# JNP-Solutions/Slacken

Hardware: AMD Instinct MI355X
Metric: classify_throughput_150bp_standard224scale (higher is better)
Workload: dtype u64

## Files before the change

### slacken_amd/csrc/lane.hip

```cpp
#include "engine.h"

#include <algorithm>
#include <cstddef>
#include <cstdio>
#include <cstdlib>

namespace slk {

#ifndef SLK_LANE_LW
#define SLK_LANE_LW 4
#endif
constexpr int LW = SLK_LANE_LW;
constexpr int QCAP = 128;
#ifndef SLK_SBLK
#define SLK_SBLK 5
#endif
constexpr int SBLK = SLK_SBLK;
#ifndef SLK_OMAP
#define SLK_OMAP 12
#endif
constexpr int OMAP = SLK_OMAP;
constexpr int OMAP_CNT_BITS = 10;
constexpr uint32_t OMAP_CNT_MASK = (1u << OMAP_CNT_BITS) - 1;

struct __attribute__((aligned(16))) LaneLds {
  uint64_t q_key[QCAP];
  uint32_t q_meta[QCAP];
  uint64_t stash[128];
  uint32_t found[64];
  uint4 sbuf[(SBLK - 1) * 64];
  uint32_t omap[OMAP * 64];
  uint32_t o_flags[64];
  uint64_t rb[64];
  uint16_t q_ord[QCAP];
};

#ifdef SLK_TUNING
#define SLK_TUNE(...) __VA_ARGS__
#define SLK_TUNE_ON(bit) ((dbg & (bit)) != 0)
#else
#define SLK_TUNE(...)
#define SLK_TUNE_ON(bit) false
#endif

#ifndef SLK_PROBE_NT
#define SLK_PROBE_NT 0
#endif
__device__ __forceinline__ ulonglong2 SLK_PROBE_LOAD(const ulonglong2 *p) {
#if SLK_PROBE_NT
  ulonglong2 v;
  v.x = __builtin_nontemporal_load(&p->x);
  v.y = __builtin_nontemporal_load(&p->y);
  return v;
#else
  return *p;
#endif
}

template <bool LONG>
__device__ __forceinline__ void fold_hit(LaneLds *L, uint32_t *ocnt, bool in, uint32_t meta, int32_t taxon) {
  if (in && taxon != 0) {
    const int owner = meta & 63;
    const int32_t kmers = (int32_t)((meta >> 7) & 0x1FFF);
    if (meta & 64) atomicAdd(&L->o_flags[owner], 1u);
    uint32_t slot = (uint32_t)(((uint64_t)((uint32_t)taxon * 0x9E3779B1u) * (uint32_t)OMAP) >> 32);
    int p = 0;
    if (LONG) {
      for (; p < OMAP; p++) {
        uint32_t old = atomicCAS(&L->omap[slot * 64 + owner], 0u, (uint32_t)taxon);
        if (old == 0u || old == (uint32_t)taxon) { atomicAdd(&ocnt[slot * 64 + owner], (uint32_t)kmers); break; }
        slot = (slot + 1 == (uint32_t)OMAP) ? 0u : slot + 1;
      }
    } else {
      const uint32_t fresh = ((uint32_t)taxon << OMAP_CNT_BITS) | (uint32_t)kmers;
      for (; p < OMAP; p++) {
        uint32_t old = atomicCAS(&L->omap[slot * 64 + owner], 0u, fresh);
        if (old == 0u) break;
        if ((old >> OMAP_CNT_BITS) == (uint32_t)taxon) { atomicAdd(&L->omap[slot * 64 + owner], (uint32_t)kmers); break; }
        slot = (slot + 1 == (uint32_t)OMAP) ? 0u : slot + 1;
      }
    }
    if (p == OMAP) atomicOr(&L->o_flags[owner], 0x80000000u);
  }
}

constexpr int PG = 64 / LPB;
template <bool HITS, bool LONG>
__device__ __forceinline__ int probe_batch(LaneLds *L, uint32_t *ocnt, const TableView &T, int qhead, int qn, int cnt, int lane, int dbg,
                                           int32_t *hit_meta, int32_t *hit_taxon) {
  const uint64_t NO_TAG = ~0ULL;
  const bool in = lane < cnt;
  const int qi = (qhead + lane) & (QCAP - 1);
  const uint64_t key = L->q_key[qi];
  const uint32_t meta = L->q_meta[qi];
  const uint32_t ord = HITS ? L->q_ord[qi] : 0u;
  const uint64_t h = fmix64(key);
  uint32_t home;
  uint64_t rem_hi;
  table_slot(T.g, h, home, rem_hi);
  uint4 st;
  const uint32_t disp = (meta >> 20) & 255;
  st.x = table_bucket(T.g, home, disp);
  st.y = 0;
  const uint64_t tag = in ? (rem_hi + disp) : NO_TAG;
  st.z = (uint32_t)tag; st.w = (uint32_t)(tag >> 32);
  ((uint4 *)L->stash)[lane] = st;
  L->found[lane] = 0;
  wave_sync();
  const int g = lane / LPB, c = lane % LPB;
  const uint64_t tmask = (1ULL << T.g.taxon_bits) - 1;
  const char *cellbase = (const char *)T.cells + c * 16;
  ulonglong2 cell[LPB];
#pragma unroll
  for (int s = 0; s < LPB; s++) {
    uint32_t bkt = ((const uint4 *)L->stash)[s * PG + g].x;
    SLK_TUNE(if (dbg & 4) bkt &= 1023u;)
    cell[s] = SLK_PROBE_LOAD((const ulonglong2 *)(cellbase + ((uint64_t)bkt << BUCKET_SHIFT)));
  }
  constexpr uint64_t GROUP_LSB = LPB == 4 ? 0x1111111111111111ULL : 0x0101010101010101ULL;
  int requeued = 0;
#pragma unroll
  for (int s = 0; s < LPB; s++) {
    const uint2 tg = *(const uint2 *)&((const uint4 *)L->stash)[s * PG + g].z;
    const uint64_t want = ((uint64_t)tg.y << 32) | tg.x;
    const bool act = want != NO_TAG;
    const bool e0 = cell[s].x == 0, e1 = cell[s].y == 0;
    const bool m0 = act && !e0 && cell_tag(T.g, cell[s].x) == want;
    const bool m1 = act && !e1 && cell_tag(T.g, cell[s].y) == want;
    if (m0 || m1) L->found[s * PG + g] = (uint32_t)((m0 ? cell[s].x : cell[s].y) & tmask);
    const bool closed = T.g.flag != 0 && c == 0 && (cell[s].x & T.g.flag) == 0;
    const uint64_t B = __ballot(m0 || m1 || e0 || e1 || !act || closed);
    uint64_t any = B;
#pragma unroll
    for (int i = 1; i < LPB; i <<= 1) any |= any >> i;
    if ((any & GROUP_LSB) != GROUP_LSB) {
      const int qj = (qhead + s * PG + g) & (QCAP - 1);
      const uint32_t m_old = L->q_meta[qj];
      const bool again = c == 0 && ((B >> (g * LPB)) & ((1u << LPB) - 1)) == 0 && (int)((m_old >> 20) & 255) < T.max_disp;
      const uint64_t k_old = L->q_key[qj];
      const uint16_t o_old = HITS ? L->q_ord[qj] : (uint16_t)0;
      const uint64_t R = __ballot(again);
      wave_sync();
      if (again) {
        const int slot = (qhead + qn + requeued + __builtin_amdgcn_mbcnt_hi((uint32_t)(R >> 32), __builtin_amdgcn_mbcnt_lo((uint32_t)R, 0))) & (QCAP - 1);
        L->q_key[slot] = k_old;
        L->q_meta[slot] = m_old + (1u << 20);
        if (HITS) L->q_ord[slot] = o_old;
      }
      requeued += __popcll(R);
    }
  }
  wave_sync();
  const int32_t taxon = (int32_t)L->found[lane];
  if (!SLK_TUNE_ON(2)) fold_hit<LONG>(L, ocnt, in, meta, taxon);
  if (HITS && in) {
    const uint64_t at = L->rb[meta & 63] + ord;
    hit_taxon[at] = ext_taxon(T, taxon);
    hit_meta[at] = pack_meta((int32_t)((meta >> 7) & 0x1FFF), 1, (meta >> 6) & 1);
  }
  wave_sync();
  return requeued;
}

#ifndef SLK_STREAM_NT
#define SLK_STREAM_NT 0
#endif
#ifndef SLK_APPLY_ROWS
#define SLK_APPLY_ROWS 4
#endif
template <class T> __device__ __forceinline__ T SLK_STREAM_LOAD(const T *p) {
#if SLK_STREAM_NT
  return __builtin_nontemporal_load(p);
#else
  return *p;
#endif
}
template <class T> __device__ __forceinline__ void SLK_STREAM_STORE(T *p, T v) {
#if SLK_STREAM_NT
  __builtin_nontemporal_store(v, p);
#else
  *p = v;
#endif
}

__device__ __forceinline__ uint32_t shard_owner(uint64_t key, uint32_t ns) {
  const uint64_t h = fmix64(key);
  return (ns & (ns - 1)) == 0 ? (uint32_t)(h & (ns - 1)) : (uint32_t)(h % ns);
}
__device__ __forceinline__ uint64_t side_load(const ShardIO &S, uint64_t batch, int lane) {
  const uint64_t i = batch * 64 + (uint64_t)lane;
  return i < S.side_n ? (uint64_t)SLK_STREAM_LOAD(&S.side_keys[i]) : 0;
}
__device__ __forceinline__ void side_probe(LaneLds *L, const TableView &T, const ShardIO &S, int lane, uint64_t batch, uint64_t key, int dbg) {
  const uint64_t base = batch * 64;
  if (base >= S.side_n) return;
  const uint64_t i = base + (uint64_t)lane;
  const bool in = i < S.side_n;
  const uint64_t h = fmix64(key);
  uint32_t home;
  uint64_t rem_hi;
  table_slot(T.g, h, home, rem_hi);
  const uint64_t tag = in ? rem_hi : ~0ULL;
  uint4 st;
  st.x = home; st.y = 0; st.z = (uint32_t)tag; st.w = (uint32_t)(tag >> 32);
  ((uint4 *)L->stash)[lane] = st;
  L->found[lane] = 0;
  wave_sync();
  const int g = lane / LPB, c = lane % LPB;
  const uint64_t tmask = (1ULL << T.g.taxon_bits) - 1;
  const char *cellbase = (const char *)T.cells + c * 16;
  ulonglong2 cell[LPB];
#pragma unroll
  for (int s = 0; s < LPB; s++) {
    uint32_t bkt = ((const uint4 *)L->stash)[s * PG + g].x;
    SLK_TUNE(if (dbg & 4) bkt &= 1023u;)
    cell[s] = SLK_PROBE_LOAD((const ulonglong2 *)(cellbase + ((uint64_t)bkt << BUCKET_SHIFT)));
  }
  uint32_t unresolved = 0;
#pragma unroll
  for (int s = 0; s < LPB; s++) {
    const uint2 tg = *(const uint2 *)&((const uint4 *)L->stash)[s * PG + g].z;
    const uint64_t want = ((uint64_t)tg.y << 32) | tg.x;
    const bool act = want != ~0ULL;
    const bool e0 = cell[s].x == 0, e1 = cell[s].y == 0;
    const bool m0 = act && !e0 && cell_tag(T.g, cell[s].x) == want;
    const bool m1 = act && !e1 && cell_tag(T.g, cell[s].y) == want;
    if (m0 || m1) L->found[s * PG + g] = (uint32_t)((m0 ? cell[s].x : cell[s].y) & tmask);
    const bool closed = T.g.flag != 0 && c == 0 && (cell[s].x & T.g.flag) == 0;
    const uint64_t B = __ballot(m0 || m1 || e0 || e1 || !act || closed);
    if (((B >> (g * LPB)) & ((1u << LPB) - 1)) == 0) unresolved |= 1u << s;
  }
  wave_sync();
  int32_t taxon = (int32_t)L->found[lane];
  const uint32_t ur = (uint32_t)__shfl((int)unresolved, (lane % PG) * LPB);
  if (in && ((ur >> (lane / PG)) & 1)) {
    for (int d = 1; d <= T.max_disp; d++) {
      const ulonglong2 *b = (const ulonglong2 *)(T.cells + ((uint64_t)table_bucket(T.g, home, (uint32_t)d) * CELLS));
      const uint64_t want = rem_hi | (uint64_t)d;
      bool has_empty = false, closed = false;
      int32_t hit = 0;
#pragma unroll
      for (int q = 0; q < LPB; q++) {
        const ulonglong2 v = b[q];
        has_empty |= (v.x == 0) | (v.y == 0);
        if (q == 0) closed = T.g.flag != 0 && (v.x & T.g.flag) == 0;
        if (v.x != 0 && cell_tag(T.g, v.x) == want) hit = (int32_t)(v.x & tmask);
        if (v.y != 0 && cell_tag(T.g, v.y) == want) hit = (int32_t)(v.y & tmask);
      }
      if (hit) { taxon = hit; break; }
      if (has_empty || closed) break;
    }
  }
  if (in && !SLK_TUNE_ON(128)) SLK_STREAM_STORE(&S.side_out[i], ext_taxon(T, taxon));
  wave_sync();
}

template <bool HITS>
__device__ __forceinline__ void apply_rows(LaneLds *L, const ApplyJob &J, int lane, uint64_t row0, uint32_t nrows) {
  const uint32_t ns = (uint32_t)J.n_shards;
  constexpr int U = SLK_APPLY_ROWS;
  for (uint32_t b = 0; b < nrows; b += U) {
    uint64_t at[U];
    bool in[U];
#pragma unroll
    for (int u = 0; u < U; u++) {
      in[u] = false;
      at[u] = 0;
      if (b + u < nrows) {
        uint32_t off = 0;
        for (uint32_t sh = 0; sh < ns; sh++) {
          const uint4 e = J.batch_log[(row0 + b + u) * ns + sh];
          const uint32_t cnt = e.z;
          if (cnt == 0) continue;
          if ((uint32_t)lane >= off && (uint32_t)lane < off + cnt) {
            in[u] = true;
            const uint32_t i = (uint32_t)lane - off;
            at[u] = (uint64_t)sh * J.cap + (i < e.w ? e.x + i : e.y + (i - e.w));
          }
          off += cnt;
        }
      }
    }
    uint32_t meta[U];
    int32_t taxon[U];
#pragma unroll
    for (int u = 0; u < U; u++) {
      meta[u] = in[u] ? SLK_STREAM_LOAD(&J.send_meta[at[u]]) : 0u;
      taxon[u] = in[u] ? SLK_STREAM_LOAD(&J.taxa[at[u]]) : 0;
    }
#pragma unroll
    for (int u = 0; u < U; u++) {
      if (b + u < nrows) {
        int32_t t = taxon[u];
        if (in[u]) {
          if (HITS) {
            const uint64_t hat = L->rb[meta[u] & 63] + (meta[u] >> 20);
            J.A.span_taxon[hat] = t;
            J.A.span_meta[hat] = pack_meta((int32_t)((meta[u] >> 7) & 0x1FFF), 1, (meta[u] >> 6) & 1);
          }
          if (J.to_dense != nullptr && t > 0) t = t < J.n_to_dense ? J.to_dense[t] : 0;
        }
        fold_hit<false>(L, nullptr, in[u], meta[u], t);
      }
    }
    wave_sync();
  }
}

template <bool HITS>
__device__ __forceinline__ void emit_batch(LaneLds *L, const FusedArgs &A, const ShardIO &S, const ApplyJob &J, int qhead, int cnt, int lane,
                                           uint64_t row, uint64_t tile, uint32_t &ch_pos, uint32_t &ch_end, uint32_t &side_j, uint64_t &side_key, int dbg) {
  SLK_TUNE(if (dbg & 256) return;)
  const bool in = lane < cnt;
  const int qi = (qhead + lane) & (QCAP - 1);
  const uint64_t key = L->q_key[qi];
  const uint32_t meta = L->q_meta[qi] | (HITS ? (uint32_t)L->q_ord[qi] << 20 : 0u);
  const uint32_t ns = (uint32_t)S.n_shards;
  const uint32_t g = ns == 1 ? 0u : shard_owner(key, ns);
  uint32_t mycount = 0, rank = 0;
  for (uint32_t sh = 0; sh < ns; sh++) {
    const uint64_t m = __ballot(in && g == sh);
    if ((uint32_t)lane == sh) mycount = (uint32_t)__popcll(m);
    if (g == sh) rank = __builtin_amdgcn_mbcnt_hi((uint32_t)(m >> 32), __builtin_amdgcn_mbcnt_lo((uint32_t)m, 0));
  }
  const uint32_t pos = ch_pos, room = ch_end - ch_pos;
  const bool need = (uint32_t)lane < ns && mycount > room;
  unsigned long long got = 0;
  if (need) got = atomicAdd(&S.cursors[lane], (unsigned long long)S.chunk);
  if (side_j < S.side_per_tile) {
    const uint64_t batch = tile * S.side_per_tile + side_j;
    const uint64_t k_now = side_key;
    side_j++;
    if (side_j < S.side_per_tile) side_key = side_load(S, batch + 1, lane);
    side_probe(L, A.T, S, lane, batch, k_now, dbg);
  }
  uint32_t fresh = 0xFFFFFFFFu;
  if (need) {
    if (got + S.chunk <= S.cap) fresh = (uint32_t)got;
    else atomicOr(A.status, 2);
  }
  if ((uint32_t)lane < ns) {
    S.batch_log[row * ns + (uint32_t)lane] = make_uint4(pos, fresh, mycount, room);
    if (need) { ch_pos = fresh == 0xFFFFFFFFu ? 0u : fresh + (mycount - room); ch_end = fresh == 0xFFFFFFFFu ? 0u : fresh + S.chunk; }
    else ch_pos = pos + mycount;
  }
  const uint32_t gpos = (uint32_t)__shfl((int)pos, (int)g), groom = (uint32_t)__shfl((int)room, (int)g), gfresh = (uint32_t)__shfl((int)fresh, (int)g);
  if (in) {
    const bool tail = rank >= groom;
    if ((!tail || gfresh != 0xFFFFFFFFu) && !SLK_TUNE_ON(32)) {
      const uint64_t at = (uint64_t)g * S.cap + (tail ? gfresh + (rank - groom) : gpos + rank);
      SLK_STREAM_STORE(&S.send_keys[at], (int64_t)key);
      SLK_STREAM_STORE(&S.send_meta[at], meta);
    }
  }
  wave_sync();
}

#ifndef SLK_PACKED_STREAM
#define SLK_PACKED_STREAM 1
#endif
#ifndef SLK_PACK_ROUNDS
#define SLK_PACK_ROUNDS 2
#endif
constexpr uint32_t PACK_MAX_SPAN = 10880;
constexpr uint32_t PACK_WORDS = PACK_MAX_SPAN / 16 + 1;
constexpr int PACK_LOADS = (PACK_MAX_SPAN + 1023) / 1024;
static_assert((size_t)PACK_WORDS * 6 <= (size_t)(SBLK - 1) * 64 * 16, "the packed tile lives in the lane-wise stream's LDS slots");
__device__ __forceinline__ void pack16(const uint4 v, uint32_t &codes, uint32_t &valid) {
  const uint32_t VM = (1u << 1) | (1u << 3) | (1u << 7) | (1u << 20) | (1u << 21);
  const uint32_t w[4] = {v.x, v.y, v.z, v.w};
  codes = 0; valid = 0;
#pragma unroll
  for (int d = 0; d < 4; d++) {
    uint32_t t = (w[d] >> 1) & 0x03030303u;
    t ^= (t >> 1) & 0x01010101u;
    t = (t | (t >> 6) | (t >> 12) | (t >> 18)) & 0xFFu;
    codes |= t << (8 * d);
#pragma unroll
    for (int b = 0; b < 4; b++) {
      const uint32_t c = (w[d] >> (8 * b)) & 0xFFu;
      const uint32_t ok = (((c & 0xC0u) == 0x40u) ? 1u : 0u) & (VM >> (c & 31u));
      valid |= (ok & 1u) << (4 * d + b);
    }
  }
}
__device__ __forceinline__ uint2 packed_take(const uint32_t *pcodes, const uint16_t *pvalid, uint32_t s) {
  const uint32_t wi = s >> 4, bo = s & 15u;
  const uint64_t c64 = (uint64_t)pcodes[wi] | ((uint64_t)pcodes[wi + 1] << 32);
  const uint32_t v32 = (uint32_t)pvalid[wi] | ((uint32_t)pvalid[wi + 1] << 16);
  return make_uint2((uint32_t)(c64 >> (2 * bo)), (v32 >> bo) & 0xFFFFu);
}

#ifndef SLK_LANE_WPS
#define SLK_LANE_WPS 0
#endif
#if SLK_LANE_WPS > 0
#define LANE_BOUNDS __launch_bounds__(LW * 64, SLK_LANE_WPS)
#else
#define LANE_BOUNDS __launch_bounds__(LW * 64) __attribute__((amdgpu_waves_per_eu(4)))
#endif

__device__ __forceinline__ int route_by_length(uint64_t len, uint32_t long_max, uint32_t b0, uint32_t b1, uint32_t b2, uint32_t seg_min_len,
                                               uint32_t wave_min, uint32_t wave_ratio_q10) {
  if (long_max != 0 && len <= long_max) return (len > b0) + (len > b1) + (len > b2);
  if (seg_min_len != 0 && len >= seg_min_len) return HandOn::SEG;
  int c = HandOn::WAVE_CLASSES - 1;
  for (uint64_t b = ((uint64_t)wave_min * wave_ratio_q10) >> 10; c > 0 && len >= b; b = (b * wave_ratio_q10) >> 10) c--;
  return HandOn::WAVE0 + c;
}
__device__ __attribute__((noinline)) void hand_on(unsigned long long *hdr, uint32_t *lists, uint64_t stride, uint64_t long_cap, uint32_t long_max,
                                                  uint32_t b0, uint32_t b1, uint32_t b2, uint32_t seg_min_len, uint32_t wave_min,
                                                  uint32_t wave_ratio_q10, const uint64_t *offsets, const uint64_t *mate_offsets, bool dfr,
                                                  bool too_long, uint64_t r, int lane, bool from_long) {
  const uint64_t DM = __ballot(dfr);
  int route = from_long ? HandOn::LATE : HandOn::REST;
  if (!from_long && dfr && too_long) {
    uint64_t len = offsets[r + 1] - offsets[r];
    if (mate_offsets) len += mate_offsets[r + 1] - mate_offsets[r];
    route = route_by_length(len, long_max, b0, b1, b2, seg_min_len, wave_min, wave_ratio_q10);
  }
  if (!from_long && lane == 0) atomicAdd(&hdr[HandOn::HANDED], (unsigned long long)__popcll(DM));
  for (int l = from_long ? HandOn::LATE : 0; l <= HandOn::LATE; l++) {
    const uint64_t M = __ballot(dfr && route == l);
    if (M == 0) continue;
    const int leader = __ffsll((long long)M) - 1;
    unsigned long long at = 0;
    if (lane == leader) at = atomicAdd(&hdr[HandOn::count_word(l)], (unsigned long long)__popcll(M));
    at = readlane64(at, leader);
    if (dfr && route == l)
      lists[HandOn::list_at(l, stride, long_cap) + at + __builtin_amdgcn_mbcnt_hi((uint32_t)(M >> 32), __builtin_amdgcn_mbcnt_lo((uint32_t)M, 0))] = (uint32_t)r;
  }
}

__global__ void __launch_bounds__(256) route_kernel(FusedArgs A) {
  constexpr int PER = 8, NL = HandOn::LISTS;
  __shared__ uint32_t cnt[NL];
  __shared__ unsigned long long base[NL];
  const uint64_t chunk = 256 * PER, chunks = (A.R + chunk - 1) / chunk;
  for (uint64_t c = blockIdx.x; c < chunks; c += gridDim.x) {
    if (threadIdx.x < NL) cnt[threadIdx.x] = 0;
    __syncthreads();
    int route[PER];
    uint32_t rank[PER];
#pragma unroll
    for (int j = 0; j < PER; j++) {
      const uint64_t r = c * chunk + (uint64_t)j * 256 + threadIdx.x;
      route[j] = -1;
      rank[j] = 0;
      if (r < A.R) {
        uint64_t len = A.offsets[r + 1] - A.offsets[r];
        if (A.mate_offsets) len += A.mate_offsets[r + 1] - A.mate_offsets[r];
        route[j] = len <= 1000 ? (int)HandOn::SHORT : route_by_length(len, A.long_max, A.long_bound[0], A.long_bound[1], A.long_bound[2],
                                                                      A.seg_min_len, A.wave_min, A.wave_ratio_q10);
        rank[j] = atomicAdd(&cnt[route[j]], 1u);
      }
    }
    __syncthreads();
    if (threadIdx.x < NL && cnt[threadIdx.x] != 0)
      base[threadIdx.x] = atomicAdd(&A.hand_hdr[HandOn::count_word((int)threadIdx.x)], (unsigned long long)cnt[threadIdx.x]);
    if (threadIdx.x == 0) {
      uint32_t handed = 0;
      for (int l = 0; l < NL; l++) if (l != HandOn::SHORT) handed += cnt[l];
      if (handed) atomicAdd(&A.hand_hdr[HandOn::HANDED], (unsigned long long)handed);
    }
    __syncthreads();
#pragma unroll
    for (int j = 0; j < PER; j++)
      if (route[j] >= 0)
        A.hand_lists[HandOn::list_at(route[j], A.hand_stride, A.hand_long_cap) + base[route[j]] + rank[j]] =
            (uint32_t)(c * chunk + (uint64_t)j * 256 + threadIdx.x);
    __syncthreads();
  }
}
void launch_route(const FusedArgs &A, hipStream_t s) {
  if (A.R == 0) return;
  hipLaunchKernelGGL(route_kernel, dim3((unsigned)std::min<uint64_t>((A.R + 2047) / 2048, 2048)), dim3(256), 0, s, A);
}

template <bool HITS, bool LONG>
__device__ __forceinline__ void resolve_lane(LaneLds *L, uint32_t *ocnt, const FusedArgs &A, int lane, uint64_t r, uint32_t oflags, int32_t total,
                                             int32_t nhits, int32_t np, int dbg) {
  const int32_t nd = (int32_t)oflags;
  uint32_t *const ecnt = LONG ? ocnt : L->omap;
  int D = 0;
  for (int s = 0; s < OMAP; s++) {
    const uint32_t e = L->omap[s * 64 + lane];
    if (e != 0) {
      if (LONG) ocnt[D * 64 + lane] = ocnt[s * 64 + lane];
      L->omap[D * 64 + lane] = e;
      D++;
    }
  }
#define ENT_TAXON(j) (LONG ? (int32_t)L->omap[(j) * 64 + lane] : (int32_t)(L->omap[(j) * 64 + lane] >> OMAP_CNT_BITS))
#define ENT_COUNT(j) (LONG ? (int32_t)ecnt[(j) * 64 + lane] : (int32_t)(ecnt[(j) * 64 + lane] & OMAP_CNT_MASK))
  int32_t maxTaxon = D ? ENT_TAXON(0) : 0;
  const int32_t c0 = D ? ENT_COUNT(0) : 0;
  uint32_t *const tin = (uint32_t *)L, *const tout = tin + OMAP * 64;
  static_assert(offsetof(LaneLds, omap) >= 2 * OMAP * 64 * sizeof(uint32_t), "the intervals alias the queue and the read stream's slots");
  uint32_t m_in = 0, m_out = 0;
  int32_t sum_all = c0;
  if (D >= 2 && !SLK_TUNE_ON(16)) {
#pragma unroll
    for (int j = 0; j < OMAP; j++) {
      if (j < D) {
        const uint4 nj = tax_node(A.nodes, A.ntax, ENT_TAXON(j));
        tin[j * 64 + lane] = nj.y;
        tout[j * 64 + lane] = nj.z;
      }
    }
    maxTaxon = 0;
    sum_all = 0;
    int32_t best = 0;
    for (int a = 0; a < D; a++) {
      const uint32_t ain = tin[a * 64 + lane], aout = tout[a * 64 + lane];
      int32_t score = 0;
      for (int b = 0; b < D; b++)
        score += (tin[b * 64 + lane] <= ain && ain <= tout[b * 64 + lane]) ? ENT_COUNT(b) : 0;
      sum_all += ENT_COUNT(a);
      if (score > best) {
        maxTaxon = ENT_TAXON(a); best = score; m_in = ain; m_out = aout;
      } else if (score == best) {
        if (m_in <= ain && ain <= m_out) {
        } else if (ain <= m_in && m_in <= aout) {
          maxTaxon = ENT_TAXON(a); m_in = ain; m_out = aout;
        } else {
          int32_t x = (int32_t)tax_node(A.nodes, A.ntax, maxTaxon).x;
          uint4 nx = make_uint4(0, 0, 0, 0);
          while (x != 0) {
            nx = tax_node(A.nodes, A.ntax, x);
            if (nx.y <= ain && ain <= nx.z) break;
            x = (int32_t)nx.x;
          }
          if (x == 0) { x = 1; nx = tax_node(A.nodes, A.ntax, 1); }
          maxTaxon = x; m_in = nx.y; m_out = nx.z;
        }
      }
    }
  }
  for (int32_t c = 0; c < A.C; c++) {
    const double required = ceil(__dmul_rn(A.thr.v[c], (double)total));
    int32_t mt = maxTaxon;
    if (D < 2 || SLK_TUNE_ON(16)) {
      if ((double)c0 < required) mt = 0;
    } else {
      uint32_t cin = m_in, cout = m_out;
      uint4 cur = make_uint4(0, 0, 0, 0);
      bool have_cur = false;
      while (mt != 0) {
        int32_t ms = 0;
        bool side = false;
        int up = -1;
        uint32_t up_in = 0;
        for (int j = 0; j < D; j++) {
          const uint32_t jin = tin[j * 64 + lane], jout = tout[j * 64 + lane];
          const bool inside = cin <= jin && jin <= cout;
          ms += inside ? ENT_COUNT(j) : 0;
          const bool above = !inside && jin <= cin && cin <= jout;
          side = side || (!inside && !above);
          if (above && (up < 0 || jin > up_in)) { up = j; up_in = jin; }
        }
        if ((double)ms >= required) break;
        if (ms == sum_all) { mt = 0; break; }
        if (!side) {
          mt = ENT_TAXON(up); cin = up_in; cout = tout[up * 64 + lane];
          have_cur = false;
        } else {
          if (!have_cur) cur = tax_node(A.nodes, A.ntax, mt);
          mt = (int32_t)cur.x;
          if (mt != 0) { cur = tax_node(A.nodes, A.ntax, mt); have_cur = true; cin = cur.y; cout = cur.z; }
        }
      }
    }
    bool classified = (mt != 0) && (nd >= A.min_hit_groups);
    A.out_taxon[(uint64_t)c * A.out_stride + r] = classified ? ext_taxon(A.T, mt) : 0;
    A.out_classified[(uint64_t)c * A.out_stride + r] = classified ? 1 : 0;
  }
#undef ENT_TAXON
#undef ENT_COUNT
  if (A.out_nd) A.out_nd[r] = nd;
  if (A.out_tk) A.out_tk[r] = total;
  if (A.out_nh) A.out_nh[r] = nhits;
  if (HITS) A.span_count[r] = nhits;
  if (A.out_np) A.out_np[r] = np;
}

template <bool W5, int MODE, bool HITS, bool LONG>
__device__ __forceinline__ void lane_body(const FusedArgs &A, const ShardIO &S, const ApplyJob *Jp, int32_t *defer, uint32_t max_len, int dbg) {
  extern __shared__ __attribute__((aligned(16))) unsigned char lds_raw[];
  const int lane = threadIdx.x & 63;
  const int wib = __builtin_amdgcn_readfirstlane(threadIdx.x >> 6);
  const ScanParams P = A.P;
  const int k = P.k, m = P.m, w = P.w;
  const size_t fixed = HITS ? sizeof(LaneLds) : offsetof(LaneLds, rb);
  const size_t win_bytes = W5 ? 0 : (size_t)w * 64 * sizeof(uint64_t);
  const size_t per_wave = fixed + win_bytes + (LONG ? (size_t)OMAP * 64 * sizeof(uint32_t) : 0);
  LaneLds *L = (LaneLds *)(lds_raw + (size_t)wib * per_wave);
  uint64_t *win = (uint64_t *)((unsigned char *)L + fixed);
  uint32_t *ocnt = LONG ? (uint32_t *)((unsigned char *)L + fixed + win_bytes) : nullptr;
  const bool paired = A.mate_bases != nullptr;
  const bool scans = MODE != LANE_EMIT || A.R != 0;
  const uint64_t bases_end = scans ? A.offsets[A.R] : 0, mates_end = (scans && paired) ? A.mate_offsets[A.R] : 0;
  uint64_t cls_n[5] = {0, 0, 0, 0, 0}, cls_tiles[5] = {0, 0, 0, 0, 0};
  uint64_t ntiles = (A.R + 63) / 64;
  if (LONG) {
    ntiles = 0;
#pragma unroll
    for (int c = 0; c < 5; c++) {
      cls_n[c] = c == 0 ? (A.route_first ? A.hand_hdr[HandOn::N_SHORT] : 0ULL) : A.hand_hdr[c - 1];
      cls_tiles[c] = (cls_n[c] + 63) / 64;
      ntiles += cls_tiles[c];
    }
  }
  const uint64_t nwaves = (uint64_t)gridDim.x * LW;
  const uint64_t etiles = ntiles;
  const uint64_t atiles = MODE == LANE_EMIT ? (Jp->A.R + 63) / 64 : 0;
  if (MODE == LANE_EMIT) ntiles = max(etiles, atiles);
  uint32_t ch_pos = 0, ch_end = 0;

  for (uint64_t tile = (uint64_t)blockIdx.x * LW + wib, it = 0;; it++) {
    if (LONG) {
      if (it) {
        unsigned long long t = 0;
        if (lane == 0) t = atomicAdd(&A.hand_hdr[HandOn::LONG_DRAW], 1ULL);
        tile = nwaves + readlane64(t, 0);
      }
    } else if (MODE == LANE_EMIT) {
      if (it) {
        unsigned long long t = 0;
        if (lane == 0) t = atomicAdd(&S.cursors[S.n_shards], 1ULL);
        tile = nwaves + readlane64(t, 0);
      }
    } else if (it) {
      tile += nwaves;
    }
    if (tile >= ntiles) break;
    uint64_t unit = tile * 64 + lane;
    bool have = unit < A.R;
    uint64_t r = unit;
    if (LONG) {
      uint64_t local = tile;
      int c = 4;
#pragma unroll
      for (int i = 4; i > 0; i--) if (c == i && local >= cls_tiles[i]) { local -= cls_tiles[i]; c = i - 1; }
      unit = local * 64 + lane;
      have = unit < cls_n[c];
      const uint32_t *const cl = A.hand_lists + HandOn::list_at(c == 0 ? (int)HandOn::SHORT : c - 1, A.hand_stride, A.hand_long_cap);
      r = have ? (uint64_t)cl[unit] : 0;
    }
    const uint8_t *seq = A.bases;
    uint32_t n = 0, n2 = 0;
    uint32_t room = 0;
    if (have) {
      uint64_t o = A.offsets[r];
      seq = A.bases + o;
      n = (uint32_t)(A.offsets[r + 1] - o);
      room = clamp_room(bases_end - o);
      SLK_TUNE(if (dbg & 8) { seq = A.bases + A.offsets[r & 1023]; room = clamp_room(bases_end - A.offsets[r & 1023]); })
      if (paired) n2 = (uint32_t)(A.mate_offsets[r + 1] - A.mate_offsets[r]);
    }
    bool too_long = have && ((uint64_t)n + n2 > max_len);
    bool fin = !have || too_long;
    uint64_t row = 0, row0 = 0;
    if (MODE == LANE_EMIT && tile < etiles) row = row0 = (span_region(A.offsets, A.mate_offsets, tile * 64) >> 6) + tile;
    const uint64_t rbase = (HITS && have) ? span_region(A.offsets, A.mate_offsets, r) : 0;
    if (HITS && MODE != LANE_EMIT) L->rb[lane] = rbase;
#pragma unroll
    for (int s = 0; s < OMAP; s++) L->omap[s * 64 + lane] = 0;
    if (LONG) {
#pragma unroll
      for (int s = 0; s < OMAP; s++) ocnt[s * 64 + lane] = 0;
    }
    L->o_flags[lane] = 0;
    if (MODE == LANE_EMIT && tile < atiles) {
      const uint64_t r2 = tile * 64 + lane;
      const bool have2 = r2 < Jp->A.R;
      const uint2 tr = Jp->tile_rows[tile];
      if (HITS) L->rb[lane] = have2 ? span_region(Jp->A.offsets, Jp->A.mate_offsets, r2) : 0;
      wave_sync();
      apply_rows<HITS>(L, *Jp, lane, tr.x, tr.y);
      const bool dfr2 = have2 && (Jp->defer[r2] != 0 || (L->o_flags[lane] & 0x80000000u));
      const uint64_t DM = __ballot(dfr2);
      if (DM != 0 && lane == 0) atomicAdd(Jp->n_deferred, (unsigned long long)__popcll(DM));
      if (have2) {
        if (dfr2) {
          Jp->defer[r2] = 1;
          if (Jp->A.out_nh) Jp->A.out_nh[r2] = 0;
          if (HITS) Jp->A.span_count[r2] = 0;
        } else {
          const int2 ri = Jp->read_info[r2];
          resolve_lane<HITS, false>(L, nullptr, Jp->A, lane, r2, L->o_flags[lane], ri.x, ri.y, 0, dbg);
        }
      }
      wave_sync();
    }
    uint32_t pos = 0;
    int mate = 0;
    uint32_t cur = 0, b1 = 0, b2 = 0, b3 = 0;
    int sb = 1;
    bool packed = false;
    uint32_t s0 = 0;
    uint32_t *const pcodes = (uint32_t *)L->sbuf;
    uint16_t *const pvalid = (uint16_t *)(pcodes + PACK_WORDS);
    constexpr bool CAN_PACK = SLK_PACKED_STREAM && !LONG && MODE == LANE_LOCAL;
    if (CAN_PACK && !paired) {
      const uint64_t t0 = tile * 64, t1 = min(A.R, t0 + 64);
      const uint64_t span_o = A.offsets[t0], span = A.offsets[t1] - span_o;
      if (span <= PACK_MAX_SPAN && __ballot(!fin) != 0) {
        packed = true;
        s0 = have ? (uint32_t)(A.offsets[r] - span_o) : 0;
        const uint8_t *tb = A.bases + span_o;
        const uint32_t troom = clamp_room(bases_end - span_o), sp = (uint32_t)span;
        constexpr int PG0 = (PACK_LOADS + SLK_PACK_ROUNDS - 1) / SLK_PACK_ROUNDS;
#pragma unroll
        for (int j0 = 0; j0 < PACK_LOADS; j0 += PG0) {
          uint4 v[PG0];
#pragma unroll
          for (int j = 0; j < PG0; j++) {
            const uint32_t cb = (uint32_t)(j0 + j) * 1024u + (uint32_t)lane * 16u;
            v[j] = make_uint4(0, 0, 0, 0);
            if (j0 + j < PACK_LOADS && cb < sp) v[j] = load_block16(tb + cb, troom - cb);
          }
#pragma unroll
          for (int j = 0; j < PG0; j++) {
            const uint32_t cb = (uint32_t)(j0 + j) * 1024u + (uint32_t)lane * 16u;
            if (j0 + j < PACK_LOADS && cb < sp + 16u) {
              uint32_t cw, vw;
              pack16(v[j], cw, vw);
              pcodes[cb >> 4] = cw;
              pvalid[cb >> 4] = (uint16_t)vw;
            }
          }
        }
        wave_sync();
      }
    }
    if (!fin && n > 0) {
      if (CAN_PACK && packed) {
        const uint2 pk = packed_take(pcodes, pvalid, s0);
        cur = pk.x; b1 = pk.y;
      } else {
        uint4 v = stream_refill<SBLK>(L, lane, seq, 0, n, room);
        cur = v.x; b1 = v.y; b2 = v.z; b3 = v.w;
      }
    }
    int run_class = 0;
    uint32_t run_len = 0, nvalid = 0;
    uint64_t fwd = 0, rc = 0;
    uint64_t k1 = ~0ULL, p1 = ~0ULL, p2 = ~0ULL, m41 = ~0ULL;
    uint64_t pre = ~0ULL;
    uint64_t cur_val = 0;
    int32_t cur_run = 0;
    bool first = true, have_last = false;
    uint64_t last_key = 0;
    int32_t total = 0, np = 0, nhits = 0;
    uint32_t side_j = (MODE == LANE_EMIT && S.side_n != 0 && tile < etiles) ? 0u : 0xFFFFFFFFu;
    uint64_t side_key = (MODE == LANE_EMIT && S.side_n != 0 && S.side_per_tile != 0 && tile < etiles) ? side_load(S, tile * S.side_per_tile, lane) : 0;
    int qn = 0;
    int qhead = 0;
    int tphase = 0;

    const uint32_t VM = (1u << 1) | (1u << 3) | (1u << 7) | (1u << 20) | (1u << 21);
    while (__ballot(!fin) != 0) {
      if (!W5 && tphase == 0) pre = ~0ULL;
      const bool act = !fin;
      const bool is_end = pos >= n;
      bool okc;
      uint32_t t;
      if (CAN_PACK && packed) {
        t = cur & 3u;
        okc = (b1 & 1u) != 0;
      } else {
        const uint32_t c = cur & 0xFF;
        okc = ((c & 0xC0) == 0x40) && ((VM >> (c & 31)) & 1);
        t = (c >> 1) & 3;
        t ^= t >> 1;
      }
      const int cls = is_end ? -1 : (okc ? 1 : 0);
      const bool run_end = act && run_len > 0 && cls != run_class;
      const bool seqrun = run_class == 1 && nvalid >= (uint32_t)k;
      const bool seq_close = run_end && seqrun;
      const bool amb_close = run_end && !seqrun && run_len >= (uint32_t)k;
      const int32_t ord0 = nhits;
      total += amb_close ? (int32_t)run_len - (k - 1) : 0;
      if (HITS && amb_close) {
        A.span_meta[rbase + ord0] = pack_meta((int32_t)run_len - (k - 1), 2, 0);
        A.span_taxon[rbase + ord0] = -1;
      }
      nhits += amb_close ? 1 : 0;
      first = first && !amb_close;
      const uint64_t ekey = cur_val;
      const int32_t ekmers = cur_run;
      run_len = run_end ? 0u : run_len;
      const bool proc = act && !is_end;
      const bool new_run = proc && run_len == 0;
      run_class = new_run ? cls : run_class;
      nvalid = new_run ? 0u : nvalid;
      cur_run = (new_run || seq_close) ? 0 : cur_run;
      run_len += proc ? 1u : 0u;
      const bool nt = proc && okc;
      nvalid += nt ? 1u : 0u;
      fwd = (fwd << 2) | ((uint64_t)t << P.sh);
      rc = ((rc >> 2) | ((uint64_t)(3 - t) << 62)) & P.keep;
      const bool havekey = nt && nvalid >= (uint32_t)m;
      const uint64_t canon = (P.canonical && rc < fwd) ? rc : fwd;
      const uint64_t key = (canon ^ P.xmask) & P.smask;
      uint64_t minv;
      if (W5) {
        const uint64_t p = umin64(key, k1);
        const uint64_t m4 = umin64(p, p2);
        minv = umin64(key, m41);
        k1 = key; p2 = p1; p1 = p; m41 = m4;
      } else {
        const uint64_t kk = havekey ? key : ~0ULL;
        pre = umin64(pre, kk);
        minv = (tphase == w - 1) ? pre : umin64(pre, win[(tphase + 1) * 64 + lane]);
        win[tphase * 64 + lane] = kk;
      }
      const bool havewin = havekey && nvalid >= (uint32_t)k;
      const bool start = havewin && cur_run == 0;
      const bool same = havewin && cur_run != 0 && minv == cur_val;
      const bool change = havewin && cur_run != 0 && minv != cur_val;
      const bool emit = seq_close || change;
      cur_val = (start || change) ? minv : cur_val;
      cur_run = (start || change) ? 1 : (same ? cur_run + 1 : cur_run);
      pos += proc ? 1u : 0u;
      const bool refill = proc && (pos & 15) == 0;
      if (CAN_PACK && packed) {
        cur = proc ? (cur >> 2) : cur;
        b1 = proc ? (b1 >> 1) : b1;
        if (__ballot(refill) != 0) {
          if (refill && pos < n) {
            const uint2 pk = packed_take(pcodes, pvalid, s0 + pos);
            cur = pk.x; b1 = pk.y;
          }
        }
      } else {
        const bool nextdw = proc && (pos & 3) == 0;
        cur = nextdw ? b1 : (proc ? (cur >> 8) : cur);
        b1 = nextdw ? b2 : b1;
        b2 = nextdw ? b3 : b2;
        if (__ballot(refill) != 0) {
          if (refill) {
            if (pos < n) {
              uint4 v;
              if (sb < SBLK) { v = L->sbuf[(sb - 1) * 64 + lane]; sb++; }
              else { v = stream_refill<SBLK>(L, lane, seq, pos, n, room); sb = 1; }
              cur = v.x; b1 = v.y; b2 = v.z; b3 = v.w;
            }
          }
        }
      }
      const bool at_end = act && is_end;
      if (__ballot(at_end) != 0) {
        if (at_end) {
          if (mate == 0 && paired) {
            if (HITS) {
              const int32_t ordb = ord0 + ((amb_close || emit) ? 1 : 0);
              A.span_meta[rbase + ordb] = pack_meta(-(k - 1), 3, 0);
              A.span_taxon[rbase + ordb] = -2;
            }
            nhits++;
            first = false;
            mate = 1;
            const uint64_t o2 = A.mate_offsets[r];
            seq = A.mate_bases + o2; n = (uint32_t)(A.mate_offsets[r + 1] - o2); room = clamp_room(mates_end - o2); pos = 0;
            if (n > 0) {
              uint4 v = stream_refill<SBLK>(L, lane, seq, 0, n, room);
              sb = 1;
              cur = v.x; b1 = v.y; b2 = v.z; b3 = v.w;
            }
          } else {
            fin = true;
          }
        }
      }
      if (!W5) {
        if (tphase == w - 1) {
          uint64_t sm = ~0ULL;
          for (int j = w - 1; j >= 0; j--) { sm = umin64(sm, win[j * 64 + lane]); win[j * 64 + lane] = sm; }
          tphase = 0;
        } else {
          tphase++;
        }
      }
      const bool distinct = emit && (first || !(have_last && ekey == last_key));
      last_key = emit ? ekey : last_key;
      have_last = have_last || emit;
      first = first && !emit;
      total += emit ? ekmers : 0;
      np += emit ? 1 : 0;
      nhits += emit ? 1 : 0;
      uint64_t E = __ballot(emit);
      if (E != 0) {
        if (emit) {
          int slot = (qhead + qn + __builtin_amdgcn_mbcnt_hi((uint32_t)(E >> 32), __builtin_amdgcn_mbcnt_lo((uint32_t)E, 0))) & (QCAP - 1);
          L->q_key[slot] = ekey;
          if (HITS) L->q_ord[slot] = (uint16_t)ord0;
          L->q_meta[slot] = (uint32_t)lane | (distinct ? 64u : 0u) | ((uint32_t)ekmers << 7);
        }
        qn += __popcll(E);
        while (qn >= 64) {
          wave_sync();
          int back = 0;
          if (MODE == LANE_EMIT) emit_batch<HITS>(L, A, S, *Jp, qhead, 64, lane, row++, tile, ch_pos, ch_end, side_j, side_key, dbg);
          else if (!SLK_TUNE_ON(1)) back = probe_batch<HITS, LONG>(L, ocnt, A.T, qhead, qn, 64, lane, dbg, A.span_meta, A.span_taxon);
          qhead = (qhead + 64) & (QCAP - 1);
          qn += back - 64;
        }
      }
    }
    while (qn > 0) {
      wave_sync();
      const int cnt = min(qn, 64);
      int back = 0;
      if (MODE == LANE_EMIT) emit_batch<HITS>(L, A, S, *Jp, qhead, cnt, lane, row++, tile, ch_pos, ch_end, side_j, side_key, dbg);
      else if (!SLK_TUNE_ON(1)) back = probe_batch<HITS, LONG>(L, ocnt, A.T, qhead, qn, cnt, lane, dbg, A.span_meta, A.span_taxon);
      qhead = (qhead + cnt) & (QCAP - 1);
      qn += back - cnt;
    }
    wave_sync();
    if (MODE == LANE_EMIT) {
      if (tile < etiles) {
        if (have) S.read_info[r] = make_int2(total, nhits);
        if (lane == 0) S.tile_rows[tile] = make_uint2((uint32_t)row0, (uint32_t)(row - row0));
      }
      while (side_j < S.side_per_tile) {
        const uint64_t batch = tile * S.side_per_tile + side_j;
        const uint64_t k_now = side_key;
        side_j++;
        if (side_j < S.side_per_tile) side_key = side_load(S, batch + 1, lane);
        side_probe(L, A.T, S, lane, batch, k_now, dbg);
      }
    }

    if (MODE == LANE_LOCAL) {
      const uint32_t oflags = have ? L->o_flags[lane] : 0u;
      const bool dfr = have && (too_long || (oflags & 0x80000000u));
      if (__ballot(dfr) != 0)
        hand_on(A.hand_hdr, A.hand_lists, A.hand_stride, A.hand_long_cap, A.long_max, A.long_bound[0], A.long_bound[1], A.long_bound[2],
                A.seg_min_len, A.wave_min, A.wave_ratio_q10, A.offsets, A.mate_offsets, dfr, too_long, r, lane, LONG);
      if (have && !dfr) resolve_lane<HITS, LONG>(L, ocnt, A, lane, r, oflags, total, nhits, np, dbg);
    } else {
      if (have && too_long) defer[r] = 1;
    }
    wave_sync();
  }
  if (MODE == LANE_EMIT) {
    for (uint32_t sh = 0; sh < (uint32_t)S.n_shards; sh++) {
      const uint32_t p0 = __builtin_amdgcn_readlane(ch_pos, sh), p1 = __builtin_amdgcn_readlane(ch_end, sh);
      for (uint32_t i = p0 + (uint32_t)lane; i < p1; i += 64) S.send_keys[(uint64_t)sh * S.cap + i] = 0;
    }
  }
}

template <bool W5, int MODE, bool HITS, bool LONG>
__global__ void LANE_BOUNDS lane_kernel(FusedArgs A, ShardIO S, int32_t *defer, uint32_t max_len, int dbg) {
  lane_body<W5, MODE, HITS, LONG>(A, S, nullptr, defer, max_len, dbg);
}
template <bool W5, bool HITS>
__global__ void LANE_BOUNDS lane_step_kernel(FusedArgs A, ShardIO S, ApplyJob J, int32_t *defer, uint32_t max_len, int dbg) {
  lane_body<W5, LANE_EMIT, HITS, false>(A, S, &J, defer, max_len, dbg);
}

static size_t lane_lds_per_wave(bool hits, bool w5, int w, bool lng) {
  return (hits ? sizeof(LaneLds) : offsetof(LaneLds, rb)) + (w5 ? 0 : (size_t)w * 64 * sizeof(uint64_t)) + (lng ? (size_t)OMAP * 64 * sizeof(uint32_t) : 0);
}

template <bool HITS, bool LONG>
static void launch_lane_mode(const FusedArgs &A, int32_t *defer, uint32_t max_len, hipStream_t s) {
  if (A.R == 0) return;
  const bool w5 = A.P.w == 5;
  const size_t per_wave = lane_lds_per_wave(HITS, w5, A.P.w, LONG);
  static const int extra_lds = (int)env_long("SLK_LANE_EXTRA_LDS", 0);
  size_t lds = per_wave * LW + (size_t)extra_lds;
  uint64_t tiles = (A.R + 63) / 64;
  uint64_t blocks = (tiles + LW - 1) / LW;
  static const int bpc = (int)env_long("SLK_LANE_BLOCKS_PER_CU", 0);
  if (bpc > 0 && blocks > (uint64_t)256 * bpc) blocks = (uint64_t)256 * bpc;
  if (LONG && blocks > 256 * 5) blocks = 256 * 5;
  dim3 g((unsigned)blocks), b(LW * 64);
#ifdef SLK_TUNING
  static const int dbg = (int)env_long("SLK_DEBUG_ABLATE", 0);
#else
  const int dbg = 0;
#endif
  static bool occ_printed = false;
  if (getenv("SLK_DEBUG_OCC") && !occ_printed) {
    occ_printed = true;
    int nb = 0;
    (void)hipOccupancyMaxActiveBlocksPerMultiprocessor(&nb, w5 ? (const void *)lane_kernel<true, LANE_LOCAL, HITS, LONG> : (const void *)lane_kernel<false, LANE_LOCAL, HITS, LONG>, LW * 64, lds);
    fprintf(stderr, "[slk] lane kernel: %zu B LDS per block, %d blocks (%d waves) resident per CU\n", lds, nb, nb * LW);
  }
  if (w5) hipLaunchKernelGGL((lane_kernel<true, LANE_LOCAL, HITS, LONG>), g, b, lds, s, A, ShardIO{}, defer, max_len, dbg);
  else hipLaunchKernelGGL((lane_kernel<false, LANE_LOCAL, HITS, LONG>), g, b, lds, s, A, ShardIO{}, defer, max_len, dbg);
}

void launch_lane(const FusedArgs &A, int32_t *defer, uint32_t max_len, hipStream_t s) {
  if (A.span_taxon) launch_lane_mode<true, false>(A, defer, max_len, s);
  else launch_lane_mode<false, false>(A, defer, max_len, s);
}
void launch_lane_long(const FusedArgs &A, uint32_t max_len, hipStream_t s) {
  if (A.span_taxon) launch_lane_mode<true, true>(A, nullptr, max_len, s);
  else launch_lane_mode<false, true>(A, nullptr, max_len, s);
}

template <bool W5, bool HITS>
static void launch_step_mode(const FusedArgs &A, const ShardIO &S, const ApplyJob &J, int32_t *defer, uint32_t max_len, hipStream_t s) {
  const uint64_t tiles = std::max((A.R + 63) / 64, (J.A.R + 63) / 64);
  if (tiles == 0) return;
  const size_t lds = lane_lds_per_wave(HITS, W5, A.P.w, false) * LW;
  static int resident[2][2] = {{0, 0}, {0, 0}};
  static int cus = 0;
  if (cus == 0) {
    int dev = 0;
    (void)hipGetDevice(&dev);
    if (hipDeviceGetAttribute(&cus, hipDeviceAttributeMultiprocessorCount, dev) != hipSuccess || cus <= 0) cus = 256;
  }
  int nb = W5 ? resident[1][HITS] : 0;
  if (nb == 0) {
    if (hipOccupancyMaxActiveBlocksPerMultiprocessor(&nb, (const void *)lane_step_kernel<W5, HITS>, LW * 64, lds) != hipSuccess || nb <= 0) nb = 4;
    if (W5) resident[1][HITS] = nb;
  }
  static const int bpc = (int)env_long("SLK_STEP_BLOCKS_PER_CU", 0);
  if (bpc > 0) nb = bpc;
  const uint64_t blocks = std::min<uint64_t>((tiles + LW - 1) / LW, (uint64_t)cus * nb);
#ifdef SLK_TUNING
  static const int dbg = (int)env_long("SLK_DEBUG_ABLATE", 0);
#else
  const int dbg = 0;
#endif
  hipLaunchKernelGGL((lane_step_kernel<W5, HITS>), dim3((unsigned)blocks), dim3(LW * 64), lds, s, A, S, J, defer, max_len, dbg);
}
void launch_lane_step(const FusedArgs &A, const ShardIO &S, const ApplyJob &J, int32_t *defer, uint32_t max_len, hipStream_t s) {
  const bool hits = A.R ? A.span_taxon != nullptr : J.A.span_taxon != nullptr;
  if (A.P.w == 5) { if (hits) launch_step_mode<true, true>(A, S, J, defer, max_len, s); else launch_step_mode<true, false>(A, S, J, defer, max_len, s); }
  else { if (hits) launch_step_mode<false, true>(A, S, J, defer, max_len, s); else launch_step_mode<false, false>(A, S, J, defer, max_len, s); }
}

}
```

Before: 1142.

## Defer unresolved side-key probes to an LDS carry queue and resolve them cooperatively

Side-key lookups that miss their home bucket are no longer handled by a divergent per-lane displacement loop. They are compacted into a carry area in LDS (reusing the taxon-map slots) and later resolved in cooperative, wave-wide bucket-probe passes, one displacement per pass. The aim is to replace serial divergent global loads with coalesced multi-lane bucket probes. The cost is extra LDS traffic, extra flush passes, and reliance on the omap region being free during emit mode. It also adds tuning counters for how many lookups stay unresolved.

```diff
diff --git a/slacken_amd/csrc/lane.hip b/slacken_amd/csrc/lane.hip
--- a/slacken_amd/csrc/lane.hip
+++ b/slacken_amd/csrc/lane.hip
@@ -191,9 +191,77 @@
   const uint64_t i = batch * 64 + (uint64_t)lane;
   return i < S.side_n ? (uint64_t)SLK_STREAM_LOAD(&S.side_keys[i]) : 0;
 }
-__device__ __forceinline__ void side_probe(LaneLds *L, const TableView &T, const ShardIO &S, int lane, uint64_t batch, uint64_t key, int dbg) {
+constexpr int CARRY_CAP = 192;
+static_assert((size_t)CARRY_CAP * sizeof(uint4) <= sizeof(LaneLds::omap), "the carry area lives in the taxon map's slots");
+static_assert(CARRY_CAP >= 128 && CARRY_CAP % 64 == 0, "room for a batch that is put aside whole, flushed in rounds of 64");
+static_assert(offsetof(LaneLds, omap) % sizeof(uint4) == 0, "16-byte entries");
+struct SideCarry {
+  uint32_t n;
+  SLK_TUNE(uint32_t seen; uint32_t unresolved;)
+};
+#ifdef SLK_TUNING
+__device__ unsigned long long slk_tune_lookups[2];
+#endif
+
+__device__ __forceinline__ void side_flush(LaneLds *L, const TableView &T, const ShardIO &S, int lane, uint64_t first, uint32_t &fill, int dbg) {
+  uint4 *const area = (uint4 *)L->omap;
+  const int g = lane / LPB, c = lane % LPB;
+  const uint64_t tmask = (1ULL << T.g.taxon_bits) - 1;
+  const uint32_t dmask = (1u << T.g.disp_bits) - 1;
+  const char *cellbase = (const char *)T.cells + c * 16;
+  uint32_t n = fill;
+  for (int pass = 0; pass < T.max_disp && n != 0; pass++) {
+    uint32_t kept = 0;
+    for (uint32_t r0 = 0; r0 < n; r0 += 64) {
+      L->found[lane] = 0;
+      wave_sync();
+      ulonglong2 cell[LPB];
+#pragma unroll
+      for (int s = 0; s < LPB; s++) {
+        const uint32_t e = r0 + s * PG + g;
+        const uint2 hz = make_uint2(area[e].x, area[e].z);
+        uint32_t bkt = e < n ? table_bucket(T.g, hz.x, hz.y & dmask) : 0u;
+        SLK_TUNE(if (dbg & 4) bkt &= 1023u;)
+        cell[s] = SLK_PROBE_LOAD((const ulonglong2 *)(cellbase + ((uint64_t)bkt << BUCKET_SHIFT)));
+      }
+      uint32_t unresolved = 0;
+#pragma unroll
+      for (int s = 0; s < LPB; s++) {
+        const uint32_t e = r0 + s * PG + g;
+        const uint2 tg = *(const uint2 *)&area[e].z;
+        const uint64_t want = ((uint64_t)tg.y << 32) | tg.x;
+        const bool act = e < n;
+        const bool e0 = cell[s].x == 0, e1 = cell[s].y == 0;
+        const bool m0 = act && !e0 && cell_tag(T.g, cell[s].x) == want;
+        const bool m1 = act && !e1 && cell_tag(T.g, cell[s].y) == want;
+        if (m0 || m1) L->found[s * PG + g] = (uint32_t)((m0 ? cell[s].x : cell[s].y) & tmask);
+        const bool closed = T.g.flag != 0 && c == 0 && (cell[s].x & T.g.flag) == 0;
+        const uint64_t B = __ballot(m0 || m1 || e0 || e1 || !act || closed);
+        if (((B >> (g * LPB)) & ((1u << LPB) - 1)) == 0) unresolved |= 1u << s;
+      }
+      wave_sync();
+      const bool in = r0 + (uint32_t)lane < n;
+      const uint4 en = area[r0 + lane];
+      const int32_t taxon = (int32_t)L->found[lane];
+      const uint32_t ur = (uint32_t)__shfl((int)unresolved, (lane % PG) * LPB);
+      const bool again = in && ((ur >> (lane / PG)) & 1) && (en.z & dmask) < (uint32_t)T.max_disp;
+      const uint64_t K = __ballot(again);
+      wave_sync();
+      if (again) area[kept + __builtin_amdgcn_mbcnt_hi((uint32_t)(K >> 32), __builtin_amdgcn_mbcnt_lo((uint32_t)K, 0))] = make_uint4(en.x, en.y, en.z + 1, en.w);
+      else if (in && !SLK_TUNE_ON(128)) SLK_STREAM_STORE(&S.side_out[first + en.y], ext_taxon(T, taxon));
+      kept += (uint32_t)__popcll(K);
+    }
+    wave_sync();
+    n = kept;
+  }
+  fill = 0;
+}
+
+__device__ __forceinline__ void side_probe(LaneLds *L, const TableView &T, const ShardIO &S, int lane, uint64_t batch, uint64_t first, uint64_t key,
+                                           SideCarry &C, int dbg) {
   const uint64_t base = batch * 64;
   if (base >= S.side_n) return;
+  if (__builtin_expect(C.n > (uint32_t)(CARRY_CAP - 64), 0)) side_flush(L, T, S, lane, first, C.n, dbg);
   const uint64_t i = base + (uint64_t)lane;
   const bool in = i < S.side_n;
   const uint64_t h = fmix64(key);
@@ -231,27 +299,21 @@
     if (((B >> (g * LPB)) & ((1u << LPB) - 1)) == 0) unresolved |= 1u << s;
   }
   wave_sync();
-  int32_t taxon = (int32_t)L->found[lane];
+  const int32_t taxon = (int32_t)L->found[lane];
   const uint32_t ur = (uint32_t)__shfl((int)unresolved, (lane % PG) * LPB);
-  if (in && ((ur >> (lane / PG)) & 1)) {
-    for (int d = 1; d <= T.max_disp; d++) {
-      const ulonglong2 *b = (const ulonglong2 *)(T.cells + ((uint64_t)table_bucket(T.g, home, (uint32_t)d) * CELLS));
-      const uint64_t want = rem_hi | (uint64_t)d;
-      bool has_empty = false, closed = false;
-      int32_t hit = 0;
-#pragma unroll
-      for (int q = 0; q < LPB; q++) {
-        const ulonglong2 v = b[q];
-        has_empty |= (v.x == 0) | (v.y == 0);
-        if (q == 0) closed = T.g.flag != 0 && (v.x & T.g.flag) == 0;
-        if (v.x != 0 && cell_tag(T.g, v.x) == want) hit = (int32_t)(v.x & tmask);
-        if (v.y != 0 && cell_tag(T.g, v.y) == want) hit = (int32_t)(v.y & tmask);
-      }
-      if (hit) { taxon = hit; break; }
-      if (has_empty || closed) break;
-    }
-  }
-  if (in && !SLK_TUNE_ON(128)) SLK_STREAM_STORE(&S.side_out[i], ext_taxon(T, taxon));
+  const bool open = in && ((ur >> (lane / PG)) & 1);
+  SLK_TUNE(C.seen += (uint32_t)__popcll(__ballot(in)); C.unresolved += (uint32_t)__popcll(__ballot(open));)
+  const bool aside = open && T.max_disp > 0 && !SLK_TUNE_ON(64);
+  const uint64_t U = __ballot(aside);
+  if (in && !aside && !SLK_TUNE_ON(128)) SLK_STREAM_STORE(&S.side_out[i], ext_taxon(T, taxon));
+  if (U != 0) {
+    if (aside) {
+      const uint64_t next = rem_hi | 1ULL;
+      ((uint4 *)L->omap)[C.n + __builtin_amdgcn_mbcnt_hi((uint32_t)(U >> 32), __builtin_amdgcn_mbcnt_lo((uint32_t)U, 0))] =
+          make_uint4(home, (uint32_t)(i - first), (uint32_t)next, (uint32_t)(next >> 32));
+    }
+    C.n += (uint32_t)__popcll(U);
+  }
   wave_sync();
 }
 
@@ -309,7 +371,7 @@
 
 template <bool HITS>
 __device__ __forceinline__ void emit_batch(LaneLds *L, const FusedArgs &A, const ShardIO &S, const ApplyJob &J, int qhead, int cnt, int lane,
-                                           uint64_t row, uint64_t tile, uint32_t &ch_pos, uint32_t &ch_end, uint32_t &side_j, uint64_t &side_key, int dbg) {
+                                           uint64_t row, uint64_t tile, uint32_t &ch_pos, uint32_t &ch_end, uint32_t &side_j, uint64_t &side_key, SideCarry &C, int dbg) {
   SLK_TUNE(if (dbg & 256) return;)
   const bool in = lane < cnt;
   const int qi = (qhead + lane) & (QCAP - 1);
@@ -332,7 +394,7 @@
     const uint64_t k_now = side_key;
     side_j++;
     if (side_j < S.side_per_tile) side_key = side_load(S, batch + 1, lane);
-    side_probe(L, A.T, S, lane, batch, k_now, dbg);
+    side_probe(L, A.T, S, lane, batch, tile * S.side_per_tile * 64, k_now, C, dbg);
   }
   uint32_t fresh = 0xFFFFFFFFu;
   if (need) {
@@ -616,6 +678,7 @@
   const uint64_t atiles = MODE == LANE_EMIT ? (Jp->A.R + 63) / 64 : 0;
   if (MODE == LANE_EMIT) ntiles = max(etiles, atiles);
   uint32_t ch_pos = 0, ch_end = 0;
+  SideCarry carry = {};
 
   for (uint64_t tile = (uint64_t)blockIdx.x * LW + wib, it = 0;; it++) {
     if (LONG) {
@@ -753,6 +816,7 @@
     bool first = true, have_last = false;
     uint64_t last_key = 0;
     int32_t total = 0, np = 0, nhits = 0;
+    carry.n = 0;
     uint32_t side_j = (MODE == LANE_EMIT && S.side_n != 0 && tile < etiles) ? 0u : 0xFFFFFFFFu;
     uint64_t side_key = (MODE == LANE_EMIT && S.side_n != 0 && S.side_per_tile != 0 && tile < etiles) ? side_load(S, tile * S.side_per_tile, lane) : 0;
     int qn = 0;
@@ -902,7 +966,7 @@
         while (qn >= 64) {
           wave_sync();
           int back = 0;
-          if (MODE == LANE_EMIT) emit_batch<HITS>(L, A, S, *Jp, qhead, 64, lane, row++, tile, ch_pos, ch_end, side_j, side_key, dbg);
+          if (MODE == LANE_EMIT) emit_batch<HITS>(L, A, S, *Jp, qhead, 64, lane, row++, tile, ch_pos, ch_end, side_j, side_key, carry, dbg);
           else if (!SLK_TUNE_ON(1)) back = probe_batch<HITS, LONG>(L, ocnt, A.T, qhead, qn, 64, lane, dbg, A.span_meta, A.span_taxon);
           qhead = (qhead + 64) & (QCAP - 1);
           qn += back - 64;
@@ -913,7 +977,7 @@
       wave_sync();
       const int cnt = min(qn, 64);
       int back = 0;
-      if (MODE == LANE_EMIT) emit_batch<HITS>(L, A, S, *Jp, qhead, cnt, lane, row++, tile, ch_pos, ch_end, side_j, side_key, dbg);
+      if (MODE == LANE_EMIT) emit_batch<HITS>(L, A, S, *Jp, qhead, cnt, lane, row++, tile, ch_pos, ch_end, side_j, side_key, carry, dbg);
       else if (!SLK_TUNE_ON(1)) back = probe_batch<HITS, LONG>(L, ocnt, A.T, qhead, qn, cnt, lane, dbg, A.span_meta, A.span_taxon);
       qhead = (qhead + cnt) & (QCAP - 1);
       qn += back - cnt;
@@ -929,8 +993,9 @@
         const uint64_t k_now = side_key;
         side_j++;
         if (side_j < S.side_per_tile) side_key = side_load(S, batch + 1, lane);
-        side_probe(L, A.T, S, lane, batch, k_now, dbg);
-      }
+        side_probe(L, A.T, S, lane, batch, tile * S.side_per_tile * 64, k_now, carry, dbg);
+      }
+      if (carry.n != 0) side_flush(L, A.T, S, lane, tile * S.side_per_tile * 64, carry.n, dbg);
     }
 
     if (MODE == LANE_LOCAL) {
@@ -946,6 +1011,7 @@
     wave_sync();
   }
   if (MODE == LANE_EMIT) {
+    SLK_TUNE(if (lane == 0 && carry.seen != 0) { atomicAdd(&slk_tune_lookups[0], (unsigned long long)carry.seen); atomicAdd(&slk_tune_lookups[1], (unsigned long long)carry.unresolved); })
     for (uint32_t sh = 0; sh < (uint32_t)S.n_shards; sh++) {
       const uint32_t p0 = __builtin_amdgcn_readlane(ch_pos, sh), p1 = __builtin_amdgcn_readlane(ch_end, sh);
       for (uint32_t i = p0 + (uint32_t)lane; i < p1; i += 64) S.send_keys[(uint64_t)sh * S.cap + i] = 0;
@@ -1038,3 +1104,10 @@
 }
 
 }
+
+#ifdef SLK_TUNING
+extern "C" int slk_tune_lookup_counts(unsigned long long *out) {
+  if (hipDeviceSynchronize() != hipSuccess) return -1;
+  return hipMemcpyFromSymbol(out, HIP_SYMBOL(slk::slk_tune_lookups), 2 * sizeof(unsigned long long)) == hipSuccess ? 0 : -1;
+}
+#endif
```

New measurement: 1142 (median of 3 runs). Within noise of the previous version (-0.0%).
